# zzzzxxxx111/Rover-SLAM

Measured on AMD Instinct MI355X. Metric: frames/s SuperPoint+LightGlue 640x480, higher is better.
Workload: dtype f32; 1 GPU; configs[3] per GPU: 33 synthetic 640x480 u8 frames resident in HBM, SuperPoint extract (Kmax=1024, thr=0.0005) + LightGlue match of 32 consecutive pairs (9 layers, filter 0.1); 32 frames counted per GPU per step; seeded synthetic weights (centred descriptor head + calibrated LightGlue law, frames shifted by multiples of 8 px); the same resident frames every step (compute-bound path, no data-depend; frames_per_gpu=32, kmax=1024, lg_fold_wo=1, pairing=calibrated

## Files before the change

### rover-slam_amd/csrc/sp_conv.hip

```cpp
#include <stdlib.h>
#include "rfe_internal.h"

namespace rfe {

constexpr int TH = 8, TW = 32, IH = TH + 2, IW = TW + 2;
constexpr int TWS = IW;
constexpr int PLANE = IH * TWS;
constexpr int NT = CONV_NT;

constexpr int CK = CONV_CK;

size_t packed_conv3x3_count(int cin, int cout, bool pool) { return (size_t)cout * cin * 9 * (conv3x3_reads_t16(cin, cout, pool) ? 2 : 1); }

void pack_conv3x3_weights(const float* w, int cin, int cout, bool pool, std::vector<float>& out) {
    out.assign(packed_conv3x3_count(cin, cout, pool), 0.f);
    const int KCH = CK * 9;
    const int nch = cin / CK, nct = cout / NT;
    for (int ct = 0; ct < nct; ++ct)
        for (int ch = 0; ch < nch; ++ch)
            for (int kl = 0; kl < KCH; ++kl)
                for (int j = 0; j < NT; ++j) {
                    int co = ct * NT + j, ci = ch * CK + kl / 9, tap = kl % 9;
                    out[(((size_t)ct * nch + ch) * KCH + kl) * NT + j] = w[((size_t)co * cin + ci) * 9 + tap];
                }
    if (!conv3x3_reads_t16(cin, cout, pool)) return;
    float* t16 = out.data() + (size_t)cout * cin * 9;
    const int nst = cin / 16;
    for (int b = 0; b < cout / 16; ++b)
        for (int st = 0; st < nst; ++st)
            for (int g = 0; g < 9; ++g)
                for (int q = 0; q < 4; ++q)
                    for (int co = 0; co < 16; ++co)
                        for (int sq = 0; sq < 4; ++sq) {
                            const int kap = 16 * g + 4 * sq + q, ci = st * 16 + kap / 9, tap = kap % 9;
                            t16[((((((size_t)b * nst + st) * 9 + g) * 4 + q) * 16 + co) * 4) + sq] = w[((size_t)(b * 16 + co) * cin + ci) * 9 + tap];
                        }
}

__device__ __forceinline__ void conv_a_offsets(int (&aoff)[9], int h, int wave, int col) {
#pragma unroll
    for (int s = 0; s < 9; ++s) {
        const int k0 = 2 * s, k1 = 2 * s + 1;
        const int o0 = (k0 / 9) * PLANE + ((k0 % 9) / 3) * TWS + (k0 % 9) % 3;
        const int o1 = (k1 / 9) * PLANE + ((k1 % 9) / 3) * TWS + (k1 % 9) % 3;
        aoff[s] = (h ? o1 : o0) + (2 * wave) * TWS + col;
    }
}

template <int PLANE_ = PLANE, int BLK1_ = TWS>
__device__ __forceinline__ void conv_chunk_mma(const float* lds_in, const float* lds_w, const int (&aoff)[9], int boff,
                                               f32x16 (&acc)[2][2]) {
#pragma unroll 1
    for (int cp = 0; cp < CK / 2; ++cp) {
        const float* ap = lds_in + cp * 2 * PLANE_;
        const float* bp = lds_w + cp * 18 * NT + boff;
#pragma unroll
        for (int s = 0; s < 9; ++s) {
            const float a0 = ap[aoff[s]], a1 = ap[aoff[s] + BLK1_];
            const float b0 = bp[2 * s * NT], b1 = bp[2 * s * NT + 32];
            acc[0][0] = __builtin_amdgcn_mfma_f32_32x32x2f32(a0, b0, acc[0][0], 0, 0, 0);
            acc[0][1] = __builtin_amdgcn_mfma_f32_32x32x2f32(a0, b1, acc[0][1], 0, 0, 0);
            acc[1][0] = __builtin_amdgcn_mfma_f32_32x32x2f32(a1, b0, acc[1][0], 0, 0, 0);
            acc[1][1] = __builtin_amdgcn_mfma_f32_32x32x2f32(a1, b1, acc[1][1], 0, 0, 0);
        }
    }
}

__device__ __forceinline__ void conv_stage_weights(float* lds_w, const float* src_chunk, int tid) {
    constexpr int KCH = CK * 9, NTHR = 256;
    const float4* src = reinterpret_cast<const float4*>(src_chunk);
    float4* dst = reinterpret_cast<float4*>(lds_w);
#pragma unroll
    for (int it = 0; it < (KCH * NT / 4 + NTHR - 1) / NTHR; ++it)
        if (it * NTHR + tid < KCH * NT / 4) dst[it * NTHR + tid] = src[it * NTHR + tid];
}

template <bool POOL, bool RELU>
__device__ __forceinline__ void conv_store(const f32x16 (&acc)[2][2], float* __restrict__ out, int b, int H, int W, int COUT,
                                           int x0, int y0, int co0, int wave, int col, int h) {
    if (!POOL) {
        float* out_b = out + (size_t)b * H * W * COUT;
#pragma unroll
        for (int mb = 0; mb < 2; ++mb) {
            const int y = y0 + 2 * wave + mb;
            if (y >= H) continue;
#pragma unroll
            for (int r = 0; r < 16; ++r) {
                const int x = x0 + (r & 3) + 8 * (r >> 2) + 4 * h;
                if (x >= W) continue;
                float v0 = acc[mb][0][r], v1 = acc[mb][1][r];
                if (RELU) { v0 = fmaxf(v0, 0.f); v1 = fmaxf(v1, 0.f); }
                float* o = out_b + ((size_t)y * W + x) * COUT + co0 + col;
                o[0] = v0; o[32] = v1;
            }
        }
    } else {
        const int Ho = H >> 1, Wo = W >> 1;
        float* out_b = out + (size_t)b * Ho * Wo * COUT;
        const int yo = (y0 >> 1) + wave;
        if (yo < Ho) {
#pragma unroll
            for (int r = 0; r < 16; r += 2) {
                const int xo = (x0 >> 1) + ((r & 3) >> 1) + 4 * (r >> 2) + 2 * h;
                if (xo >= Wo) continue;
#pragma unroll
                for (int nb = 0; nb < 2; ++nb) {
                    float v = fmaxf(fmaxf(acc[0][nb][r], acc[0][nb][r + 1]), fmaxf(acc[1][nb][r], acc[1][nb][r + 1]));
                    if (RELU) v = fmaxf(v, 0.f);
                    out_b[((size_t)yo * Wo + xo) * COUT + co0 + nb * 32 + col] = v;
                }
            }
        }
    }
}

struct ConvBlock { int b, bx, by, ct; bool valid; };
__device__ __forceinline__ ConvBlock conv_decode(int nct, int gx, int gy, int ntiles) {
    const int L = blockIdx.x, xcd = L & 7, t = L >> 3;
    ConvBlock k;
    k.ct = t % nct;
    const int u = (t / nct) * 8 + xcd;
    k.valid = u < ntiles;
    k.bx = u % gx; k.by = (u / gx) % gy; k.b = u / (gx * gy);
    return k;
}
static inline unsigned conv_grid(int gx, int gy, int B, int nct) { return (unsigned)(((gx * gy * B + 7) / 8) * 8 * nct); }

template <int CIN, bool POOL, bool RELU, int TAG>
__global__ __launch_bounds__(256, 2) void conv3x3_mfma_kernel(
    const float* __restrict__ in, const float* __restrict__ wp, const float* __restrict__ bias,
    float* __restrict__ out, int H, int W, int COUT, int gx, int gy, int ntiles) {
    constexpr int KCH = CK * 9;
    __shared__ __attribute__((aligned(16))) float lds[CK * PLANE + KCH * NT];
    float* lds_in = lds;
    float* lds_w = lds + CK * PLANE;

    const int tid = threadIdx.x;
    const int lane = tid & 63;
    const int wave = __builtin_amdgcn_readfirstlane(tid >> 6);
    const int col = lane & 31, h = lane >> 5;
    const ConvBlock blk = conv_decode(COUT / NT, gx, gy, ntiles);
    if (!blk.valid) return;
    const int b = blk.b, ct = blk.ct;
    const int x0 = blk.bx * TW, y0 = blk.by * TH;
    const int co0 = ct * NT;

    f32x16 acc[2][2];
    {
        const float b0 = bias[co0 + col], b1 = bias[co0 + 32 + col];
#pragma unroll
        for (int r = 0; r < 16; ++r) { acc[0][0][r] = b0; acc[1][0][r] = b0; acc[0][1][r] = b1; acc[1][1][r] = b1; }
    }
    int aoff[9];
    conv_a_offsets(aoff, h, wave, col);
    const int boff = h * NT + col;

    const float* in_b = in + (size_t)b * H * W * CIN;
    const float* wp_ct = wp + (size_t)ct * (CIN / CK) * KCH * NT;

    constexpr int S_IT = (IH * IW * (CK / 4) + 255) / 256;
    int s_goff[S_IT], s_loff[S_IT];
#pragma unroll
    for (int it = 0; it < S_IT; ++it) {
        const int idx = tid + it * 256;
        const int cq = idx % (CK / 4), pix = idx / (CK / 4);
        const int py = pix / IW, px = pix % IW;
        const int gy = y0 - 1 + py, gx = x0 - 1 + px;
        const bool slot = idx < IH * IW * (CK / 4);
        s_loff[it] = slot ? (cq * 4) * PLANE + py * TWS + px : -1;
        s_goff[it] = (slot && gy >= 0 && gy < H && gx >= 0 && gx < W) ? (gy * W + gx) * CIN + cq * 4 : -1;
    }

    constexpr bool PAIR = (CIN / CK) % 2 == 0;
    float4 v_odd[S_IT];
    for (int ch = 0; ch < CIN / CK; ++ch) {
        __syncthreads();
#pragma unroll
        for (int it = 0; it < S_IT; ++it) {
            if (s_loff[it] < 0) continue;
            float4 v = make_float4(0.f, 0.f, 0.f, 0.f);
            if (!PAIR) {
                if (s_goff[it] >= 0) v = *reinterpret_cast<const float4*>(in_b + s_goff[it] + ch * CK);
            } else if ((ch & 1) == 0) {
                v_odd[it] = v;
                if (s_goff[it] >= 0) {
                    v = *reinterpret_cast<const float4*>(in_b + s_goff[it] + ch * CK);
                    v_odd[it] = *reinterpret_cast<const float4*>(in_b + s_goff[it] + (ch + 1) * CK);
                }
            } else {
                v = v_odd[it];
            }
            float* d = lds_in + s_loff[it];
            d[0] = v.x; d[PLANE] = v.y; d[2 * PLANE] = v.z; d[3 * PLANE] = v.w;
        }
        conv_stage_weights(lds_w, wp_ct + (size_t)ch * KCH * NT, tid);
        __syncthreads();
        conv_chunk_mma(lds_in, lds_w, aoff, boff, acc);
    }
    conv_store<POOL, RELU>(acc, out, b, H, W, COUT, x0, y0, co0, wave, col, h);
}

constexpr int STH = 4, SNT = 32;

template <int CIN, bool RELU, bool POOL = false>
__global__ __launch_bounds__(64 * STH, 4) void conv3x3_small_kernel(
    const float* __restrict__ in, const float* __restrict__ wp, const float* __restrict__ bias,
    float* __restrict__ out, int H, int W, int COUT, int gx, int gy, int ntiles) {
    constexpr int KCH = CK * 9;
    constexpr int NTH = 64 * STH, RIH = STH + 2, RPLANE = RIH * TWS;
    constexpr int LDS_WORDS = (CK * RPLANE + KCH * SNT) > (POOL ? STH * TW * SNT : 0) ? (CK * RPLANE + KCH * SNT) : STH * TW * SNT;
    __shared__ __attribute__((aligned(16))) float lds[LDS_WORDS];
    float* lds_in = lds;
    float* lds_w = lds + CK * RPLANE;
    const int tid = threadIdx.x, lane = tid & 63;
    const int wave = __builtin_amdgcn_readfirstlane(tid >> 6);
    const int col = lane & 31, h = lane >> 5;
    const ConvBlock blk = conv_decode(COUT / SNT, gx, gy, ntiles);
    if (!blk.valid) return;
    const int b = blk.b, ct = blk.ct;
    const int x0 = blk.bx * TW, y0 = blk.by * STH;
    const int co0 = ct * SNT;

    f32x16 acc;
    {
        const float b0 = bias[co0 + col];
#pragma unroll
        for (int r = 0; r < 16; ++r) acc[r] = b0;
    }
    int aoff[9];
#pragma unroll
    for (int s = 0; s < 9; ++s) {
        const int k0 = 2 * s, k1 = 2 * s + 1;
        const int o0 = (k0 / 9) * RPLANE + ((k0 % 9) / 3) * TWS + (k0 % 9) % 3;
        const int o1 = (k1 / 9) * RPLANE + ((k1 % 9) / 3) * TWS + (k1 % 9) % 3;
        aoff[s] = (h ? o1 : o0) + wave * TWS + col;
    }
    const int boff = h * SNT + col;
    const float* in_b = in + (size_t)b * H * W * CIN;
    const float* wp_ct = wp + (size_t)(ct >> 1) * (CIN / CK) * KCH * NT + (ct & 1) * SNT;

    for (int ch = 0; ch < CIN / CK; ++ch) {
        __syncthreads();
        for (int idx = tid; idx < RIH * IW * (CK / 4); idx += NTH) {
            const int cq = idx % (CK / 4), pix = idx / (CK / 4);
            const int py = pix / IW, px = pix % IW;
            const int gy = y0 - 1 + py, gx = x0 - 1 + px;
            float4 v = make_float4(0.f, 0.f, 0.f, 0.f);
            if (gy >= 0 && gy < H && gx >= 0 && gx < W)
                v = *reinterpret_cast<const float4*>(in_b + ((size_t)gy * W + gx) * CIN + ch * CK + cq * 4);
            float* d = lds_in + (cq * 4) * RPLANE + py * TWS + px;
            d[0] = v.x; d[RPLANE] = v.y; d[2 * RPLANE] = v.z; d[3 * RPLANE] = v.w;
        }
        {
            const float* src = wp_ct + (size_t)ch * KCH * NT;
            for (int idx = tid; idx < KCH * (SNT / 4); idx += NTH) {
                const int kl = idx / (SNT / 4), q = idx % (SNT / 4);
                reinterpret_cast<float4*>(lds_w)[idx] = *reinterpret_cast<const float4*>(src + kl * NT + q * 4);
            }
        }
        __syncthreads();
#pragma unroll 1
        for (int cp = 0; cp < CK / 2; ++cp) {
            const float* ap = lds_in + cp * 2 * RPLANE;
            const float* bp = lds_w + cp * 18 * SNT + boff;
#pragma unroll
            for (int s = 0; s < 9; ++s) acc = __builtin_amdgcn_mfma_f32_32x32x2f32(ap[aoff[s]], bp[2 * s * SNT], acc, 0, 0, 0);
        }
    }
    if (POOL) {
        __syncthreads();
#pragma unroll
        for (int r = 0; r < 16; ++r) {
            const int xl = (r & 3) + 8 * (r >> 2) + 4 * h;
            float v = acc[r];
            if (RELU) v = fmaxf(v, 0.f);
            lds[(wave * TW + xl) * SNT + col] = v;
        }
        __syncthreads();
        const int Ho = H >> 1, Wo = W >> 1;
        float* out_b = out + (size_t)b * Ho * Wo * COUT;
        const int chn = tid & 31;
#pragma unroll
        for (int it = 0; it < (STH / 2) * (TW / 2) / 8; ++it) {
            const int pp = (tid >> 5) + 8 * it, pr = pp / (TW / 2), pc = pp % (TW / 2);
            const int yo = (y0 >> 1) + pr, xo = (x0 >> 1) + pc;
            if (yo >= Ho || xo >= Wo) continue;
            const float* e = lds + ((2 * pr) * TW + 2 * pc) * SNT + chn;
            out_b[((size_t)yo * Wo + xo) * COUT + co0 + chn] = fmaxf(fmaxf(e[0], e[SNT]), fmaxf(e[TW * SNT], e[TW * SNT + SNT]));
        }
        return;
    }
    const int y = y0 + wave;
    if (y < H) {
        float* out_b = out + (size_t)b * H * W * COUT;
#pragma unroll
        for (int r = 0; r < 16; ++r) {
            const int x = x0 + (r & 3) + 8 * (r >> 2) + 4 * h;
            if (x >= W) continue;
            float v = acc[r];
            if (RELU) v = fmaxf(v, 0.f);
            out_b[((size_t)y * W + x) * COUT + co0 + col] = v;
        }
    }
}

constexpr int T16_H = 4, T16_W = 16, T16_IH = T16_H + 2, T16_IW = T16_W + 2, T16_PLANE = T16_IH * T16_IW, T16_NC = 32, T16_CK = 16;

typedef __attribute__((address_space(3))) void* conv_lds_ptr_t;
typedef const __attribute__((address_space(1))) void* conv_gptr_t;
constexpr int T16D_WROWS = 144, T16D_PIX = 128;
__device__ __attribute__((aligned(64))) float t16d_zero_line[16];

template <int CIN, bool RELU, int NC = T16_NC, bool POOL = false>
__global__ __launch_bounds__(256, 2) void conv3x3_t16d_kernel(
    const float* __restrict__ in, const float* __restrict__ wp, const float* __restrict__ bias,
    float* __restrict__ out, int H, int W, int COUT, int gx, int gy, int ntiles) {
    static_assert(NC == 32 || NC == 16, "32 or 16 output channels per workgroup");
    constexpr int NB = NC / 16;
    constexpr int NST = CIN / T16_CK;
    constexpr int IST_W = T16D_PIX * T16_CK, WST_W = T16D_WROWS * NC;
    extern __shared__ __attribute__((aligned(16))) float lds[];
    float* const lin = lds;
    float* const lwr = lds + 3 * IST_W;
    const int tid = threadIdx.x, lane = tid & 63;
    const int wave = __builtin_amdgcn_readfirstlane(tid >> 6);
    const int px = lane & 15, q = lane >> 4;
    const ConvBlock blk = conv_decode(COUT / NC, gx, gy, ntiles);
    if (!blk.valid) return;
    const int b = blk.b, ct = blk.ct;
    const int x0 = blk.bx * T16_W, y0 = blk.by * T16_H;
    const int co0 = ct * NC;

    f32x4 acc[NB];
#pragma unroll
    for (int nb = 0; nb < NB; ++nb) acc[nb] = *reinterpret_cast<const f32x4*>(bias + co0 + nb * 16 + 4 * q);
    int poff[4][9];
#pragma unroll
    for (int s9 = 0; s9 < 9; ++s9) {
        const int kap = 4 * s9 + q, e = kap / 9, tap = kap % 9;
        const int p = (wave + tap / 3) * T16_IW + px + tap % 3;
#pragma unroll
        for (int c4 = 0; c4 < 4; ++c4) poff[c4][s9] = p * T16_CK + e + ((c4 ^ ((p >> 2) & 3)) << 2);
    }
    const float* in_b = in + (size_t)b * H * W * CIN;
    const float* wp_t16 = wp + (size_t)COUT * CIN * 9;
    constexpr int NSLOT = 9 * NB, WCP = (NSLOT + 3) / 4, BLK_W = 9 * 256;
    int w_slot[WCP];
    const float* w_src[WCP];
#pragma unroll
    for (int u = 0; u < WCP; ++u) {
        w_slot[u] = wave + 4 * u < NSLOT ? wave + 4 * u : wave + 4 * (u - 1);
        const int nbk = w_slot[u] / 9, gs = w_slot[u] % 9;
        w_src[u] = wp_t16 + ((size_t)(ct * NB + nbk) * NST) * BLK_W + gs * 256 + lane * 4;
    }
    const float* i_src[2];
    bool i_img[2];
#pragma unroll
    for (int u = 0; u < 2; ++u) {
        const int p = (wave + 4 * u) * 16 + (lane >> 2);
        const int py = p / T16_IW, pxx = p % T16_IW;
        const int gyy = y0 - 1 + py, gxx = x0 - 1 + pxx;
        const int g = (lane & 3) ^ ((p >> 2) & 3);
        i_img[u] = p < T16_PLANE && gyy >= 0 && gyy < H && gxx >= 0 && gxx < W;
        i_src[u] = i_img[u] ? in_b + ((size_t)gyy * W + gxx) * CIN + g * 4 : t16d_zero_line + g * 4;
    }
    auto issue = [&](int st) {
        float* wdst = lwr + (st % 3) * WST_W;
        float* idst = lin + (st % 3) * IST_W;
#pragma unroll
        for (int u = 0; u < WCP; ++u)
            __builtin_amdgcn_global_load_lds((conv_gptr_t)(w_src[u] + (size_t)st * BLK_W), (conv_lds_ptr_t)(wdst + w_slot[u] * 256), 16, 0, 0);
#pragma unroll
        for (int u = 0; u < 2; ++u)
            __builtin_amdgcn_global_load_lds((conv_gptr_t)(i_src[u] + (i_img[u] ? st * T16_CK : 0)), (conv_lds_ptr_t)(idst + (wave + 4 * u) * 256), 16, 0, 0);
    };
    issue(0);
    if (NST > 1) issue(1);
    for (int st = 0; st < NST; ++st) {
        __builtin_amdgcn_sched_barrier(0);
        if (st + 1 < NST) asm volatile("s_waitcnt vmcnt(%0)\n\ts_barrier" ::"n"(WCP + 2) : "memory");
        else asm volatile("s_waitcnt vmcnt(0)\n\ts_barrier" ::: "memory");
        __builtin_amdgcn_sched_barrier(0);
        if (st + 2 < NST) issue(st + 2);
        const float* li = lin + (st % 3) * IST_W;
        const float* lw = lwr + (st % 3) * WST_W + (q * 16 + px) * 4;
#pragma unroll
        for (int g = 0; g < 9; ++g) {
            f32x4 wf[NB];
#pragma unroll
            for (int nb = 0; nb < NB; ++nb) wf[nb] = *reinterpret_cast<const f32x4*>(lw + nb * BLK_W + g * 256);
#pragma unroll
            for (int sq = 0; sq < 4; ++sq) {
                constexpr int dummy = 0; (void)dummy;
                const int s36 = 4 * g + sq;
                const float pv = li[poff[s36 / 9][s36 % 9]];
#pragma unroll
                for (int nb = 0; nb < NB; ++nb) acc[nb] = __builtin_amdgcn_mfma_f32_16x16x4f32(wf[nb][sq], pv, acc[nb], 0, 0, 0);
            }
        }
    }
    if (RELU) {
#pragma unroll
        for (int nb = 0; nb < NB; ++nb) { acc[nb][0] = fmaxf(acc[nb][0], 0.f); acc[nb][1] = fmaxf(acc[nb][1], 0.f); acc[nb][2] = fmaxf(acc[nb][2], 0.f); acc[nb][3] = fmaxf(acc[nb][3], 0.f); }
    }
    if (POOL) {
        __builtin_amdgcn_sched_barrier(0);
        asm volatile("s_waitcnt lgkmcnt(0)\n\ts_barrier" ::: "memory");
        __builtin_amdgcn_sched_barrier(0);
        float* ex = lds;
#pragma unroll
        for (int nb = 0; nb < NB; ++nb) {
            f32x4 hm;
#pragma unroll
            for (int e = 0; e < 4; ++e) hm[e] = fmaxf(acc[nb][e], __shfl_xor(acc[nb][e], 1));
            if (!(px & 1)) *reinterpret_cast<f32x4*>(ex + (wave * 8 + (px >> 1)) * NC + nb * 16 + 4 * q) = hm;
        }
        __syncthreads();
        constexpr int CG = NC / 4;
        if (tid < 2 * 8 * CG) {
            const int cg = tid % CG, ppx = (tid / CG) & 7, prow = tid / (8 * CG);
            const f32x4 a = *reinterpret_cast<const f32x4*>(ex + ((2 * prow) * 8 + ppx) * NC + cg * 4);
            const f32x4 c = *reinterpret_cast<const f32x4*>(ex + ((2 * prow + 1) * 8 + ppx) * NC + cg * 4);
            const int Ho = H >> 1, Wo = W >> 1, yo = (y0 >> 1) + prow, xo = (x0 >> 1) + ppx;
            if (yo < Ho && xo < Wo)
                *reinterpret_cast<f32x4*>(out + (((size_t)b * Ho + yo) * Wo + xo) * COUT + co0 + cg * 4) =
                    f32x4{fmaxf(a[0], c[0]), fmaxf(a[1], c[1]), fmaxf(a[2], c[2]), fmaxf(a[3], c[3])};
        }
        return;
    }
    const int y = y0 + wave, x = x0 + px;
    if (y < H && x < W) {
        float* o = out + (((size_t)b * H + y) * W + x) * COUT + co0 + 4 * q;
#pragma unroll
        for (int nb = 0; nb < NB; ++nb) *reinterpret_cast<f32x4*>(o + nb * 16) = acc[nb];
    }
}

constexpr int CIH = TH + 4, CIW = TW + 4, CPLANE = CIH * CIW;
template <int CIN, bool RELU, int TAG>
__global__ __launch_bounds__(256, 2) void conv3x3_comp_kernel(
    const float* __restrict__ in, const float* __restrict__ wp, const float* __restrict__ bias,
    float* __restrict__ out, int B, int H, int W, int COUT, int gx, int gy, int ntiles) {
    constexpr int KCH = CK * 9;
    __shared__ __attribute__((aligned(16))) float lds[CK * CPLANE + KCH * NT];
    float* lds_in = lds;
    float* lds_w = lds + CK * CPLANE;
    const int tid = threadIdx.x;
    const int lane = tid & 63;
    const int wave = __builtin_amdgcn_readfirstlane(tid >> 6);
    const int col = lane & 31, h = lane >> 5;
    const ConvBlock blk = conv_decode(COUT / NT, gx, gy, ntiles);
    if (!blk.valid) return;
    const int ct = blk.ct, co0 = ct * NT;
    const int x0 = blk.bx * TW, y0 = blk.by * TH;
    const int pair0 = y0 / H, yin = y0 % H, half0 = x0 / W, xin = x0 % W;
    const int rb = (H - yin) < TH ? (H - yin) : TH;
    const int cb = (W - xin) < TW ? (W - xin) : TW;
    auto frame_of = [&](int pr, int pc) { const int hf = half0 + pc; const int f = 2 * (pair0 + pr) + hf; return (hf <= 1 && f < B) ? f : -1; };
    if (frame_of(0, 0) < 0 && frame_of(0, 1) < 0 && frame_of(1, 0) < 0 && frame_of(1, 1) < 0) return;

    f32x16 acc[2][2];
    {
        const float b0 = bias[co0 + col], b1 = bias[co0 + 32 + col];
#pragma unroll
        for (int r = 0; r < 16; ++r) { acc[0][0][r] = b0; acc[1][0][r] = b0; acc[0][1][r] = b1; acc[1][1][r] = b1; }
    }
    int aoff[9];
    {
        const int r0 = 2 * wave;
        const int base = (r0 + (r0 >= rb ? 2 : 0)) * CIW + col + (col >= cb ? 2 : 0);
#pragma unroll
        for (int s = 0; s < 9; ++s) {
            const int k0 = 2 * s, k1 = 2 * s + 1;
            const int o0 = (k0 / 9) * CPLANE + ((k0 % 9) / 3) * CIW + (k0 % 9) % 3;
            const int o1 = (k1 / 9) * CPLANE + ((k1 % 9) / 3) * CIW + (k1 % 9) % 3;
            aoff[s] = (h ? o1 : o0) + base;
        }
    }
    const int boff = h * NT + col;
    const float* wp_ct = wp + (size_t)ct * (CIN / CK) * KCH * NT;

    constexpr int S_IT = (CIH * CIW * (CK / 4) + 255) / 256;
    int s_goff[S_IT], s_loff[S_IT];
#pragma unroll
    for (int it = 0; it < S_IT; ++it) {
        const int idx = tid + it * 256;
        const int cq = idx % (CK / 4), pix = idx / (CK / 4);
        const int lr = pix / CIW, lc = pix % CIW;
        const int pr = lr >= rb + 2, hr = lr - (pr ? rb + 2 : 0), nr = pr ? TH - rb : rb;
        const int pc = lc >= cb + 2, hc = lc - (pc ? cb + 2 : 0), nc = pc ? TW - cb : cb;
        const bool slot = idx < CIH * CIW * (CK / 4) && nr > 0 && nc > 0 && hr < nr + 2 && hc < nc + 2;
        const int y = (pr ? 0 : yin) + hr - 1, x = (pc ? 0 : xin) + hc - 1;
        const int f = frame_of(pr, pc);
        s_loff[it] = slot ? (cq * 4) * CPLANE + lr * CIW + lc : -1;
        s_goff[it] = (slot && f >= 0 && y >= 0 && y < H && x >= 0 && x < W) ? ((f * H + y) * W + x) * CIN + cq * 4 : -1;
    }
    static_assert((CIN / CK) % 2 == 0, "paired chunk fetch");
    float4 v_odd[S_IT];
    for (int ch = 0; ch < CIN / CK; ++ch) {
        __syncthreads();
#pragma unroll
        for (int it = 0; it < S_IT; ++it) {
            if (s_loff[it] < 0) continue;
            float4 v = make_float4(0.f, 0.f, 0.f, 0.f);
            if ((ch & 1) == 0) {
                v_odd[it] = v;
                if (s_goff[it] >= 0) {
                    v = *reinterpret_cast<const float4*>(in + s_goff[it] + ch * CK);
                    v_odd[it] = *reinterpret_cast<const float4*>(in + s_goff[it] + (ch + 1) * CK);
                }
            } else {
                v = v_odd[it];
            }
            float* d = lds_in + s_loff[it];
            d[0] = v.x; d[CPLANE] = v.y; d[2 * CPLANE] = v.z; d[3 * CPLANE] = v.w;
        }
        conv_stage_weights(lds_w, wp_ct + (size_t)ch * KCH * NT, tid);
        __syncthreads();
        conv_chunk_mma<CPLANE, CIW>(lds_in, lds_w, aoff, boff, acc);
    }
#pragma unroll
    for (int mb = 0; mb < 2; ++mb) {
        const int r = 2 * wave + mb, pr = r >= rb;
        const int y = pr ? r - rb : yin + r;
#pragma unroll
        for (int q = 0; q < 16; ++q) {
            const int c = (q & 3) + 8 * (q >> 2) + 4 * h, pc = c >= cb;
            const int x = pc ? c - cb : xin + c;
            const int f = frame_of(pr, pc);
            if (f < 0) continue;
            float v0 = acc[mb][0][q], v1 = acc[mb][1][q];
            if (RELU) { v0 = fmaxf(v0, 0.f); v1 = fmaxf(v1, 0.f); }
            float* o = out + (((size_t)f * H + y) * W + x) * COUT + co0 + col;
            o[0] = v0; o[32] = v1;
        }
    }
}

template <typename PX>
__device__ __forceinline__ float px_value(PX v) {
    if constexpr (sizeof(PX) == 1) return (float)v * 0.003921568859368563f;
    else return v;
}

template <typename PX>
__global__ __launch_bounds__(256, 2) void conv1ab_fused_kernel(
    const PX* __restrict__ img, int stride, const float* __restrict__ w1a , const float* __restrict__ b1a,
    const float* __restrict__ wp, const float* __restrict__ bias, float* __restrict__ out, int H, int W, long long frame_step ) {
    constexpr int CIN = 64, COUT = 64, KCH = CK * 9;
    constexpr int MH = TH + 4, MW = TW + 4;
    __shared__ __attribute__((aligned(16))) float lds[CK * PLANE + KCH * NT + MH * MW];
    float* lds_in = lds;
    float* lds_w = lds + CK * PLANE;
    float* lds_img = lds_w + KCH * NT;

    const int tid = threadIdx.x;
    const int lane = tid & 63;
    const int wave = __builtin_amdgcn_readfirstlane(tid >> 6);
    const int col = lane & 31, h = lane >> 5;
    const int b = blockIdx.z;
    const int x0 = blockIdx.x * TW, y0 = blockIdx.y * TH;

    f32x16 acc[2][2];
    {
        const float b0 = bias[col], b1 = bias[32 + col];
#pragma unroll
        for (int r = 0; r < 16; ++r) { acc[0][0][r] = b0; acc[1][0][r] = b0; acc[0][1][r] = b1; acc[1][1][r] = b1; }
    }
    int aoff[9];
    conv_a_offsets(aoff, h, wave, col);
    const int boff = h * NT + col;

    const PX* im = img + (long long)b * frame_step;
    for (int idx = tid; idx < MH * MW; idx += 256) {
        const int py = idx / MW, px = idx % MW;
        const int gy = y0 - 2 + py, gx = x0 - 2 + px;
        float v = 0.f;
        if (gy >= 0 && gy < H && gx >= 0 && gx < W) v = px_value(im[(size_t)gy * stride + gx]);
        lds_img[idx] = v;
    }

    constexpr int P_IT = (IH * IW + 255) / 256;
    int p_loff[P_IT]; bool p_inb[P_IT]; float p_iv[P_IT][9];
    __syncthreads();
#pragma unroll
    for (int it = 0; it < P_IT; ++it) {
        const int p = tid + it * 256;
        const int py = p / IW, px = p % IW;
        const int gy = y0 - 1 + py, gx = x0 - 1 + px;
        p_loff[it] = p < IH * IW ? py * TWS + px : -1;
        p_inb[it] = gy >= 0 && gy < H && gx >= 0 && gx < W;
#pragma unroll
        for (int k = 0; k < 9; ++k) p_iv[it][k] = p < IH * IW ? lds_img[(py + k / 3) * MW + px + k % 3] : 0.f;
    }

    for (int ch = 0; ch < CIN / CK; ++ch) {
        __syncthreads();
#pragma unroll
        for (int it = 0; it < P_IT; ++it) {
            if (p_loff[it] < 0) continue;
#pragma unroll
            for (int e = 0; e < CK; ++e) {
                const int c = ch * CK + e;
                float a = b1a[c];
#pragma unroll
                for (int k = 0; k < 9; ++k) a = fmaf(p_iv[it][k], w1a[k * 64 + c], a);
                lds_in[e * PLANE + p_loff[it]] = p_inb[it] ? fmaxf(a, 0.f) : 0.f;
            }
        }
        conv_stage_weights(lds_w, wp + (size_t)ch * KCH * NT, tid);
        __syncthreads();
        conv_chunk_mma(lds_in, lds_w, aoff, boff, acc);
    }
    conv_store<true, true>(acc, out, b, H, W, COUT, x0, y0, 0, wave, col, h);
}

void launch_conv1ab_fused(hipStream_t s, const void* img, bool img_f32, int stride, int B, int H, int W, const float* w1a,
                          const float* b1a, const float* wp, const float* bias, float* out, long long frame_step) {
    dim3 grid((W + TW - 1) / TW, (H + TH - 1) / TH, B);
    if (frame_step == 0) frame_step = (long long)stride * H;
    if (img_f32) hipLaunchKernelGGL((conv1ab_fused_kernel<float>), grid, dim3(256), 0, s, (const float*)img, stride, w1a, b1a, wp, bias, out, H, W, frame_step);
    else hipLaunchKernelGGL((conv1ab_fused_kernel<uint8_t>), grid, dim3(256), 0, s, (const uint8_t*)img, stride, w1a, b1a, wp, bias, out, H, W, frame_step);
}

#define RFE_CONV_LAUNCH(CIN, POOL, RELU, TAG)                                                                            \
    hipLaunchKernelGGL((conv3x3_mfma_kernel<CIN, POOL, RELU, TAG>), dim3(conv_grid(gx, gy, B, cout / NT)), dim3(256), 0, s, in, wp, bias, out, H, W, cout, gx, gy, gx * gy * B)

constexpr int CONV_T16_PX = 12000, CONV_T16_PX64 = 20000, CONV_T16P_PX128 = 20000;

bool conv3x3_reads_t16(int cin, int cout, bool pool) { return (cin == 128 || (cin == 64 && !pool)) && cout % T16_NC == 0; }

void launch_conv3x3(hipStream_t s, const float* in, int B, int H, int W, int cin, const float* wp,
                    const float* bias, int cout, bool relu, bool pool, float* out, int tag) {
    const int gx = (W + TW - 1) / TW, gy = (H + TH - 1) / TH;
    const long long px = (long long)B * H * W;
    constexpr int CONV_SMALL = 700;
    const bool small = (long long)gx * gy * B * (cout / NT) < CONV_SMALL && (cin == 64 || cin == 128);
    if (small && relu && !pool && px <= (cin == 64 ? CONV_T16_PX64 : CONV_T16_PX) && cout % T16_NC == 0) {
        const int sx = (W + T16_W - 1) / T16_W, sy = (H + T16_H - 1) / T16_H;
        constexpr int CONV_T16_NC16 = 1000;
        if (cin == 128 && (long long)sx * sy * B * (cout / T16_NC) < CONV_T16_NC16) {
            const dim3 g16(conv_grid(sx, sy, B, cout / 16));
            constexpr int b16 = 3 * (T16D_PIX * T16_CK + T16D_WROWS * 16) * 4;
            static bool l16_[64];
            ensure_dynamic_lds((const void*)conv3x3_t16d_kernel<128, true, 16>, b16, l16_);
            hipLaunchKernelGGL((conv3x3_t16d_kernel<128, true, 16>), g16, dim3(256), b16, s, in, wp, bias, out, H, W, cout, sx, sy, sx * sy * B);
            return;
        }
        const dim3 gs(conv_grid(sx, sy, B, cout / T16_NC));
        constexpr int bytes = 3 * (T16D_PIX * T16_CK + T16D_WROWS * T16_NC) * 4;
        static bool ls_[2][64];
        if (cin == 128) {
            ensure_dynamic_lds((const void*)conv3x3_t16d_kernel<128, true>, bytes, ls_[0]);
            hipLaunchKernelGGL((conv3x3_t16d_kernel<128, true>), gs, dim3(256), bytes, s, in, wp, bias, out, H, W, cout, sx, sy, sx * sy * B);
        } else {
            ensure_dynamic_lds((const void*)conv3x3_t16d_kernel<64, true>, bytes, ls_[1]);
            hipLaunchKernelGGL((conv3x3_t16d_kernel<64, true>), gs, dim3(256), bytes, s, in, wp, bias, out, H, W, cout, sx, sy, sx * sy * B);
        }
        return;
    }
    if (relu && pool && cin == 128 && px <= CONV_T16P_PX128 && cout % T16_NC == 0 && H % 2 == 0 && W % 2 == 0) {
        const int sx = (W + T16_W - 1) / T16_W, sy = (H + T16_H - 1) / T16_H;
        constexpr int b16 = 3 * (T16D_PIX * T16_CK + T16D_WROWS * 16) * 4;
        static bool lp_[64];
        ensure_dynamic_lds((const void*)conv3x3_t16d_kernel<128, true, 16, true>, b16, lp_);
        hipLaunchKernelGGL((conv3x3_t16d_kernel<128, true, 16, true>), dim3(conv_grid(sx, sy, B, cout / 16)), dim3(256), b16, s, in, wp, bias, out, H, W, cout, sx, sy, sx * sy * B);
        return;
    }
    if (small && (!pool || relu)) {
        const int sx = (W + TW - 1) / TW, sy = (H + STH - 1) / STH;
        const dim3 gs(conv_grid(sx, sy, B, cout / SNT));
        if (pool) {
            if (cin == 128) hipLaunchKernelGGL((conv3x3_small_kernel<128, true, true>), gs, dim3(256), 0, s, in, wp, bias, out, H, W, cout, sx, sy, sx * sy * B);
            else hipLaunchKernelGGL((conv3x3_small_kernel<64, true, true>), gs, dim3(256), 0, s, in, wp, bias, out, H, W, cout, sx, sy, sx * sy * B);
        }
        else if (cin == 128 && relu) hipLaunchKernelGGL((conv3x3_small_kernel<128, true>), gs, dim3(256), 0, s, in, wp, bias, out, H, W, cout, sx, sy, sx * sy * B);
        else if (cin == 128) hipLaunchKernelGGL((conv3x3_small_kernel<128, false>), gs, dim3(256), 0, s, in, wp, bias, out, H, W, cout, sx, sy, sx * sy * B);
        else if (relu) hipLaunchKernelGGL((conv3x3_small_kernel<64, true>), gs, dim3(256), 0, s, in, wp, bias, out, H, W, cout, sx, sy, sx * sy * B);
        else hipLaunchKernelGGL((conv3x3_small_kernel<64, false>), gs, dim3(256), 0, s, in, wp, bias, out, H, W, cout, sx, sy, sx * sy * B);
        return;
    }
    if (!pool && relu && cin == 128 && (tag == L_4A || tag == L_4B || tag == L_PA || tag == L_DA) && B >= 2 &&
        H % 2 == 0 && W >= TW && H >= TH && (H % TH != 0 || W % TW != 0) &&
        (long long)B * H * W * cin < (1ll << 31)) {
        const int cx = (2 * W + TW - 1) / TW, cy = (((B + 1) / 2) * H + TH - 1) / TH;
        const dim3 gc(conv_grid(cx, cy, 1, cout / NT));
        switch (tag) {
            case L_4A: hipLaunchKernelGGL((conv3x3_comp_kernel<128, true, L_4A>), gc, dim3(256), 0, s, in, wp, bias, out, B, H, W, cout, cx, cy, cx * cy); return;
            case L_4B: hipLaunchKernelGGL((conv3x3_comp_kernel<128, true, L_4B>), gc, dim3(256), 0, s, in, wp, bias, out, B, H, W, cout, cx, cy, cx * cy); return;
            case L_PA: hipLaunchKernelGGL((conv3x3_comp_kernel<128, true, L_PA>), gc, dim3(256), 0, s, in, wp, bias, out, B, H, W, cout, cx, cy, cx * cy); return;
            default: hipLaunchKernelGGL((conv3x3_comp_kernel<128, true, L_DA>), gc, dim3(256), 0, s, in, wp, bias, out, B, H, W, cout, cx, cy, cx * cy); return;
        }
    }
    switch (tag) {
        case L_2A: RFE_CONV_LAUNCH(64, false, true, L_2A); return;
        case L_2B: RFE_CONV_LAUNCH(64, true, true, L_2B); return;
        case L_3A: RFE_CONV_LAUNCH(64, false, true, L_3A); return;
        case L_3B: RFE_CONV_LAUNCH(128, true, true, L_3B); return;
        case L_4A: RFE_CONV_LAUNCH(128, false, true, L_4A); return;
        case L_4B: RFE_CONV_LAUNCH(128, false, true, L_4B); return;
        case L_PA: RFE_CONV_LAUNCH(128, false, true, L_PA); return;
        case L_DA: RFE_CONV_LAUNCH(128, false, true, L_DA); return;
        default: break;
    }
#define RFE_CONV_GEN(CIN)                                                    \
    do {                                                                     \
        if (pool && relu) RFE_CONV_LAUNCH(CIN, true, true, 0);               \
        else if (relu) RFE_CONV_LAUNCH(CIN, false, true, 0);                 \
        else if (pool) RFE_CONV_LAUNCH(CIN, true, false, 0);                 \
        else RFE_CONV_LAUNCH(CIN, false, false, 0);                          \
    } while (0)
    if (cin == 64) RFE_CONV_GEN(64);
    else if (cin == 128) RFE_CONV_GEN(128);
    else if (cin == 16) RFE_CONV_GEN(16);
    else if (cin == 32) RFE_CONV_GEN(32);
}

}
```

Measured before the change: 956.7 frames/s.

## Relayout conv LDS tiles for immediate-offset reads and software-pipeline MFMA fetches

```diff
diff --git a/rover-slam_amd/csrc/sp_conv.hip b/rover-slam_amd/csrc/sp_conv.hip
--- a/rover-slam_amd/csrc/sp_conv.hip
+++ b/rover-slam_amd/csrc/sp_conv.hip
@@ -5,10 +5,19 @@
 
 constexpr int TH = 8, TW = 32, IH = TH + 2, IW = TW + 2;
 constexpr int TWS = IW;
-constexpr int PLANE = IH * TWS;
 constexpr int NT = CONV_NT;
+typedef float f32x2 __attribute__((ext_vector_type(2)));
+typedef const volatile __attribute__((address_space(3))) f32x2* conv_lds_f32x2_t;
 
 constexpr int CK = CONV_CK;
+
+constexpr int ATW = TW + 4;
+constexpr int AROW = (CK / 2) * ATW;
+template <int ROWS>
+__host__ __device__ constexpr int conv_a_index(int ci, int row, int x) { return (ci & 1) * ROWS * AROW + row * AROW + (ci >> 1) * ATW + x; }
+template <int ROWS>
+constexpr int conv_a_words() { return 2 * ROWS * AROW; }
+static_assert((CK - 2) / 2 * ATW + AROW <= 255, "a chunk's A reads are immediates of ds_read2_b32");
 
 size_t packed_conv3x3_count(int cin, int cout, bool pool) { return (size_t)cout * cin * 9 * (conv3x3_reads_t16(cin, cout, pool) ? 2 : 1); }
 
@@ -37,42 +46,65 @@
                         }
 }
 
-__device__ __forceinline__ void conv_a_offsets(int (&aoff)[9], int h, int wave, int col) {
+template <int ROWS>
+__device__ __forceinline__ void conv_a_offsets(int (&aoff)[9], int h, int row0, int col0) {
 #pragma unroll
     for (int s = 0; s < 9; ++s) {
         const int k0 = 2 * s, k1 = 2 * s + 1;
-        const int o0 = (k0 / 9) * PLANE + ((k0 % 9) / 3) * TWS + (k0 % 9) % 3;
-        const int o1 = (k1 / 9) * PLANE + ((k1 % 9) / 3) * TWS + (k1 % 9) % 3;
-        aoff[s] = (h ? o1 : o0) + (2 * wave) * TWS + col;
-    }
-}
-
-template <int PLANE_ = PLANE, int BLK1_ = TWS>
-__device__ __forceinline__ void conv_chunk_mma(const float* lds_in, const float* lds_w, const int (&aoff)[9], int boff,
-                                               f32x16 (&acc)[2][2]) {
-#pragma unroll 1
-    for (int cp = 0; cp < CK / 2; ++cp) {
-        const float* ap = lds_in + cp * 2 * PLANE_;
-        const float* bp = lds_w + cp * 18 * NT + boff;
-#pragma unroll
-        for (int s = 0; s < 9; ++s) {
-            const float a0 = ap[aoff[s]], a1 = ap[aoff[s] + BLK1_];
-            const float b0 = bp[2 * s * NT], b1 = bp[2 * s * NT + 32];
-            acc[0][0] = __builtin_amdgcn_mfma_f32_32x32x2f32(a0, b0, acc[0][0], 0, 0, 0);
-            acc[0][1] = __builtin_amdgcn_mfma_f32_32x32x2f32(a0, b1, acc[0][1], 0, 0, 0);
-            acc[1][0] = __builtin_amdgcn_mfma_f32_32x32x2f32(a1, b0, acc[1][0], 0, 0, 0);
-            acc[1][1] = __builtin_amdgcn_mfma_f32_32x32x2f32(a1, b1, acc[1][1], 0, 0, 0);
-        }
-    }
-}
+        const int o0 = conv_a_index<ROWS>(k0 / 9, (k0 % 9) / 3, (k0 % 9) % 3);
+        const int o1 = conv_a_index<ROWS>(k1 / 9, (k1 % 9) / 3, (k1 % 9) % 3);
+        aoff[s] = (h ? o1 : o0) + conv_a_index<ROWS>(0, row0, col0);
+        asm volatile("" : "+v"(aoff[s]));
+    }
+}
+
+template <int ROWS>
+__device__ __forceinline__ void conv_a_store4(float* d, const float4& v) {
+    d[conv_a_index<ROWS>(0, 0, 0)] = v.x; d[conv_a_index<ROWS>(2, 0, 0)] = v.z;
+    d[conv_a_index<ROWS>(1, 0, 0)] = v.y; d[conv_a_index<ROWS>(3, 0, 0)] = v.w;
+}
+
+template <int ROWS>
+__device__ __forceinline__ void conv_chunk_mma(const float* lds_in, const float* lds_wl, const int (&aoff)[9], f32x16 (&acc)[2][2]) {
+    constexpr int KS = (CK / 2) * 9;
+    float a0, a1;
+    f32x2 bv;
+    auto fetch = [&](int i, float& fa0, float& fa1, f32x2& fb) {
+        const int cp = i / 9, s = i % 9;
+        fa0 = lds_in[aoff[s] + conv_a_index<ROWS>(2 * cp, 0, 0)];
+        fa1 = lds_in[aoff[s] + conv_a_index<ROWS>(2 * cp, 1, 0)];
+        fb = *((conv_lds_f32x2_t)lds_wl + (cp * 18 + 2 * s) * (NT / 2));
+    };
+    fetch(0, a0, a1, bv);
+#pragma unroll
+    for (int i = 0; i < KS; ++i) {
+        float n0 = 0.f, n1 = 0.f;
+        f32x2 nb = {0.f, 0.f};
+        if (i + 1 < KS) fetch(i + 1, n0, n1, nb);
+        acc[0][0] = __builtin_amdgcn_mfma_f32_32x32x2f32(a0, bv[0], acc[0][0], 0, 0, 0);
+        acc[0][1] = __builtin_amdgcn_mfma_f32_32x32x2f32(a0, bv[1], acc[0][1], 0, 0, 0);
+        acc[1][0] = __builtin_amdgcn_mfma_f32_32x32x2f32(a1, bv[0], acc[1][0], 0, 0, 0);
+        acc[1][1] = __builtin_amdgcn_mfma_f32_32x32x2f32(a1, bv[1], acc[1][1], 0, 0, 0);
+        __builtin_amdgcn_sched_barrier(0);
+        a0 = n0; a1 = n1; bv = nb;
+    }
+}
+__device__ __forceinline__ int conv_b_offset(int h, int col) { return h * NT + 2 * col; }
 
 __device__ __forceinline__ void conv_stage_weights(float* lds_w, const float* src_chunk, int tid) {
-    constexpr int KCH = CK * 9, NTHR = 256;
+    constexpr int KCH = CK * 9, NTHR = 256, SLOTS = KCH * (NT / 8);
     const float4* src = reinterpret_cast<const float4*>(src_chunk);
     float4* dst = reinterpret_cast<float4*>(lds_w);
 #pragma unroll
-    for (int it = 0; it < (KCH * NT / 4 + NTHR - 1) / NTHR; ++it)
-        if (it * NTHR + tid < KCH * NT / 4) dst[it * NTHR + tid] = src[it * NTHR + tid];
+    for (int it = 0; it < (SLOTS + NTHR - 1) / NTHR; ++it) {
+        const int idx = it * NTHR + tid;
+        if (idx < SLOTS) {
+            const int kl = idx / (NT / 8), q = idx % (NT / 8);
+            const float4 lo = src[kl * (NT / 4) + q], hi = src[kl * (NT / 4) + NT / 8 + q];
+            dst[2 * idx] = make_float4(lo.x, hi.x, lo.y, hi.y);
+            dst[2 * idx + 1] = make_float4(lo.z, hi.z, lo.w, hi.w);
+        }
+    }
 }
 
 template <bool POOL, bool RELU>
@@ -131,9 +163,9 @@
     const float* __restrict__ in, const float* __restrict__ wp, const float* __restrict__ bias,
     float* __restrict__ out, int H, int W, int COUT, int gx, int gy, int ntiles) {
     constexpr int KCH = CK * 9;
-    __shared__ __attribute__((aligned(16))) float lds[CK * PLANE + KCH * NT];
+    __shared__ __attribute__((aligned(16))) float lds[conv_a_words<IH>() + KCH * NT];
     float* lds_in = lds;
-    float* lds_w = lds + CK * PLANE;
+    float* lds_w = lds + conv_a_words<IH>();
 
     const int tid = threadIdx.x;
     const int lane = tid & 63;
@@ -152,8 +184,8 @@
         for (int r = 0; r < 16; ++r) { acc[0][0][r] = b0; acc[1][0][r] = b0; acc[0][1][r] = b1; acc[1][1][r] = b1; }
     }
     int aoff[9];
-    conv_a_offsets(aoff, h, wave, col);
-    const int boff = h * NT + col;
+    conv_a_offsets<IH>(aoff, h, 2 * wave, col);
+    const float* lds_wl = lds_w + conv_b_offset(h, col);
 
     const float* in_b = in + (size_t)b * H * W * CIN;
     const float* wp_ct = wp + (size_t)ct * (CIN / CK) * KCH * NT;
@@ -167,7 +199,7 @@
         const int py = pix / IW, px = pix % IW;
         const int gy = y0 - 1 + py, gx = x0 - 1 + px;
         const bool slot = idx < IH * IW * (CK / 4);
-        s_loff[it] = slot ? (cq * 4) * PLANE + py * TWS + px : -1;
+        s_loff[it] = slot ? conv_a_index<IH>(cq * 4, py, px) : -1;
         s_goff[it] = (slot && gy >= 0 && gy < H && gx >= 0 && gx < W) ? (gy * W + gx) * CIN + cq * 4 : -1;
     }
 
@@ -190,12 +222,11 @@
             } else {
                 v = v_odd[it];
             }
-            float* d = lds_in + s_loff[it];
-            d[0] = v.x; d[PLANE] = v.y; d[2 * PLANE] = v.z; d[3 * PLANE] = v.w;
+            conv_a_store4<IH>(lds_in + s_loff[it], v);
         }
         conv_stage_weights(lds_w, wp_ct + (size_t)ch * KCH * NT, tid);
         __syncthreads();
-        conv_chunk_mma(lds_in, lds_w, aoff, boff, acc);
+        conv_chunk_mma<IH>(lds_in, lds_wl, aoff, acc);
     }
     conv_store<POOL, RELU>(acc, out, b, H, W, COUT, x0, y0, co0, wave, col, h);
 }
@@ -436,15 +467,16 @@
     }
 }
 
-constexpr int CIH = TH + 4, CIW = TW + 4, CPLANE = CIH * CIW;
+constexpr int CIH = TH + 4, CIW = TW + 4;
+static_assert(CIW == ATW, "the composite tile's rows fill the LDS image's");
 template <int CIN, bool RELU, int TAG>
-__global__ __launch_bounds__(256, 2) void conv3x3_comp_kernel(
+__global__ __launch_bounds__(256, 4) void conv3x3_comp_kernel(
     const float* __restrict__ in, const float* __restrict__ wp, const float* __restrict__ bias,
     float* __restrict__ out, int B, int H, int W, int COUT, int gx, int gy, int ntiles) {
     constexpr int KCH = CK * 9;
-    __shared__ __attribute__((aligned(16))) float lds[CK * CPLANE + KCH * NT];
+    __shared__ __attribute__((aligned(16))) float lds[conv_a_words<CIH>() + KCH * NT];
     float* lds_in = lds;
-    float* lds_w = lds + CK * CPLANE;
+    float* lds_w = lds + conv_a_words<CIH>();
     const int tid = threadIdx.x;
     const int lane = tid & 63;
     const int wave = __builtin_amdgcn_readfirstlane(tid >> 6);
@@ -468,16 +500,9 @@
     int aoff[9];
     {
         const int r0 = 2 * wave;
-        const int base = (r0 + (r0 >= rb ? 2 : 0)) * CIW + col + (col >= cb ? 2 : 0);
-#pragma unroll
-        for (int s = 0; s < 9; ++s) {
-            const int k0 = 2 * s, k1 = 2 * s + 1;
-            const int o0 = (k0 / 9) * CPLANE + ((k0 % 9) / 3) * CIW + (k0 % 9) % 3;
-            const int o1 = (k1 / 9) * CPLANE + ((k1 % 9) / 3) * CIW + (k1 % 9) % 3;
-            aoff[s] = (h ? o1 : o0) + base;
-        }
-    }
-    const int boff = h * NT + col;
+        conv_a_offsets<CIH>(aoff, h, r0 + (r0 >= rb ? 2 : 0), col + (col >= cb ? 2 : 0));
+    }
+    const float* lds_wl = lds_w + conv_b_offset(h, col);
     const float* wp_ct = wp + (size_t)ct * (CIN / CK) * KCH * NT;
 
     constexpr int S_IT = (CIH * CIW * (CK / 4) + 255) / 256;
@@ -492,7 +517,7 @@
         const bool slot = idx < CIH * CIW * (CK / 4) && nr > 0 && nc > 0 && hr < nr + 2 && hc < nc + 2;
         const int y = (pr ? 0 : yin) + hr - 1, x = (pc ? 0 : xin) + hc - 1;
         const int f = frame_of(pr, pc);
-        s_loff[it] = slot ? (cq * 4) * CPLANE + lr * CIW + lc : -1;
+        s_loff[it] = slot ? conv_a_index<CIH>(cq * 4, lr, lc) : -1;
         s_goff[it] = (slot && f >= 0 && y >= 0 && y < H && x >= 0 && x < W) ? ((f * H + y) * W + x) * CIN + cq * 4 : -1;
     }
     static_assert((CIN / CK) % 2 == 0, "paired chunk fetch");
@@ -506,18 +531,19 @@
             if ((ch & 1) == 0) {
                 v_odd[it] = v;
                 if (s_goff[it] >= 0) {
-                    v = *reinterpret_cast<const float4*>(in + s_goff[it] + ch * CK);
-                    v_odd[it] = *reinterpret_cast<const float4*>(in + s_goff[it] + (ch + 1) * CK);
+                    int g = s_goff[it];
+                    asm volatile("" : "+v"(g));
+                    v = *reinterpret_cast<const float4*>(in + g + ch * CK);
+                    v_odd[it] = *reinterpret_cast<const float4*>(in + g + (ch + 1) * CK);
                 }
             } else {
                 v = v_odd[it];
             }
-            float* d = lds_in + s_loff[it];
-            d[0] = v.x; d[CPLANE] = v.y; d[2 * CPLANE] = v.z; d[3 * CPLANE] = v.w;
+            conv_a_store4<CIH>(lds_in + s_loff[it], v);
         }
         conv_stage_weights(lds_w, wp_ct + (size_t)ch * KCH * NT, tid);
         __syncthreads();
-        conv_chunk_mma<CPLANE, CIW>(lds_in, lds_w, aoff, boff, acc);
+        conv_chunk_mma<CIH>(lds_in, lds_wl, aoff, acc);
     }
 #pragma unroll
     for (int mb = 0; mb < 2; ++mb) {
@@ -549,9 +575,9 @@
     const float* __restrict__ wp, const float* __restrict__ bias, float* __restrict__ out, int H, int W, long long frame_step ) {
     constexpr int CIN = 64, COUT = 64, KCH = CK * 9;
     constexpr int MH = TH + 4, MW = TW + 4;
-    __shared__ __attribute__((aligned(16))) float lds[CK * PLANE + KCH * NT + MH * MW];
+    __shared__ __attribute__((aligned(16))) float lds[conv_a_words<IH>() + KCH * NT + MH * MW];
     float* lds_in = lds;
-    float* lds_w = lds + CK * PLANE;
+    float* lds_w = lds + conv_a_words<IH>();
     float* lds_img = lds_w + KCH * NT;
 
     const int tid = threadIdx.x;
@@ -568,8 +594,8 @@
         for (int r = 0; r < 16; ++r) { acc[0][0][r] = b0; acc[1][0][r] = b0; acc[0][1][r] = b1; acc[1][1][r] = b1; }
     }
     int aoff[9];
-    conv_a_offsets(aoff, h, wave, col);
-    const int boff = h * NT + col;
+    conv_a_offsets<IH>(aoff, h, 2 * wave, col);
+    const float* lds_wl = lds_w + conv_b_offset(h, col);
 
     const PX* im = img + (long long)b * frame_step;
     for (int idx = tid; idx < MH * MW; idx += 256) {
@@ -588,7 +614,7 @@
         const int p = tid + it * 256;
         const int py = p / IW, px = p % IW;
         const int gy = y0 - 1 + py, gx = x0 - 1 + px;
-        p_loff[it] = p < IH * IW ? py * TWS + px : -1;
+        p_loff[it] = p < IH * IW ? conv_a_index<IH>(0, py, px) : -1;
         p_inb[it] = gy >= 0 && gy < H && gx >= 0 && gx < W;
 #pragma unroll
         for (int k = 0; k < 9; ++k) p_iv[it][k] = p < IH * IW ? lds_img[(py + k / 3) * MW + px + k % 3] : 0.f;
@@ -605,12 +631,12 @@
                 float a = b1a[c];
 #pragma unroll
                 for (int k = 0; k < 9; ++k) a = fmaf(p_iv[it][k], w1a[k * 64 + c], a);
-                lds_in[e * PLANE + p_loff[it]] = p_inb[it] ? fmaxf(a, 0.f) : 0.f;
+                lds_in[conv_a_index<IH>(e, 0, 0) + p_loff[it]] = p_inb[it] ? fmaxf(a, 0.f) : 0.f;
             }
         }
         conv_stage_weights(lds_w, wp + (size_t)ch * KCH * NT, tid);
         __syncthreads();
-        conv_chunk_mma(lds_in, lds_w, aoff, boff, acc);
+        conv_chunk_mma<IH>(lds_in, lds_wl, aoff, acc);
     }
     conv_store<true, true>(acc, out, b, H, W, COUT, x0, y0, 0, wave, col, h);
 }
```

New measurement: 954.1 frames/s. No clear change (-0.3%).
